# Shigangli/Ok-Topk

Measured on AMD Instinct MI355X. Metric: tokens/s (bert_base seq128 bs8/GPU, Ok-Topk density=0.001, step time & allreduce ms; speedup vs dense), higher is better.
Workload: dtype bf16; 1 GPU; model=bert_base, global_batch=8, seq_len=128, parallelism=dp1, compressor=oktopk, wire_dtype=bf16

## Files before the change

### oktopk_amd/allreducer.py

```python
from __future__ import annotations

import logging
import math
import time
from dataclasses import dataclass
from typing import Dict, List, Optional, Tuple

import torch

from . import ops
from .comm import Comm
from .config import EngineConfig

logger = logging.getLogger("oktopk_amd")

COMPRESSORS = [
    "none",
    "dense",
    "oktopk",
    "topkA",
    "topkA2",
    "topkAopt",
    "topkSA",
    "gtopk",
    "gaussiank",
    "gaussiankconcat",
    "gaussiankSA",
]


@dataclass
class TensorState:

    residual: torch.Tensor
    counter: int = 0
    tau_local: float = 0.0
    tau_global: float = 0.0
    boundaries: Optional[torch.Tensor] = None
    mask: Optional[torch.Tensor] = None
    grad_src: Optional[torch.Tensor] = None

    def state_dict(self) -> dict:
        return {
            "residual": self.residual,
            "counter": self.counter,
            "tau_local": self.tau_local,
            "tau_global": self.tau_global,
            "boundaries": self.boundaries,
        }

    def load_state_dict(self, d: dict) -> None:
        self.residual.copy_(d["residual"].to(self.residual.device))
        self.counter = int(d["counter"])
        self.tau_local = float(d["tau_local"])
        self.tau_global = float(d["tau_global"])
        self.boundaries = d["boundaries"]


class AllReducer:

    def __init__(self, comm: Comm, cfg: Optional[EngineConfig] = None):
        self.comm = comm
        self.cfg = cfg or EngineConfig()
        if self.cfg.compressor not in COMPRESSORS:
            raise ValueError(
                f"unknown compressor {self.cfg.compressor!r}; choose from {COMPRESSORS}"
            )
        self.states: Dict[str, TensorState] = {}
        self.timers: Dict[str, Dict[str, float]] = {}
        self.eps_log: List[Tuple[int, float]] = []
        self.randk_log: List[Tuple[int, float]] = []
        self.upbound_log: List[Tuple[int, float]] = []
        self.train_epoch = 0
        self.timing_sync = False

    def set_comm(self, comm: Comm) -> None:
        self.comm = comm
        for st in self.states.values():
            st.boundaries = None

    def state(self, name: str, t: torch.Tensor) -> TensorState:
        st = self.states.get(name)
        if st is None:
            st = TensorState(residual=torch.zeros_like(t))
            self.states[name] = st
        return st

    def _time(self, name: str, phase: str, dt: float) -> None:
        self.timers.setdefault(name, {}).setdefault(phase, 0.0)
        self.timers[name][phase] += dt

    def run(self, name: str, tensor: torch.Tensor,
            grad_src: Optional[torch.Tensor] = None) -> torch.Tensor:
        t = tensor.reshape(-1)
        if self.timing_sync and t.is_cuda:
            torch.cuda.synchronize()
        comp = self.cfg.compressor
        if comp == "oktopk" and self.cfg.oktopk.pipeline_chunks > 1:
            return self._oktopk_chunked(name, tensor, grad_src)
        st = self.state(name, t)
        ok = self.cfg.oktopk
        fused_ef = comp in ("oktopk", "topkAopt", "topkSA", "gaussiankSA") or (
            self.cfg.gaussian_device_select
            and comp in ("gaussiank", "gaussiankconcat"))
        if grad_src is not None and not (
            fused_ef and st.counter >= ok.dense_warmup_iters
        ):
            t.copy_(grad_src.reshape(-1).to(t.dtype))
            grad_src = None
        st.grad_src = grad_src

        eps_ref = None
        if self.cfg.profiling_norm and comp not in ("none", "dense"):
            if grad_src is not None:
                dense_in = grad_src.reshape(-1).to(t.dtype) + st.residual
            else:
                dense_in = t + st.residual
            eps_ref = self._dense_value(dense_in)
            k = self._k(t.numel())
            top = torch.topk(eps_ref.abs(), k)
            eps_topk = torch.zeros_like(eps_ref)
            eps_topk[top.indices] = eps_ref[top.indices]
            eps_den = max(ops.l2norm(eps_ref), 1e-30)
            eps_ref = (eps_topk, eps_den, eps_ref)

        if comp in ("none", "dense") or st.counter < ok.dense_warmup_iters:
            out = self._dense(name, t)
        elif comp == "oktopk":
            out = self._oktopk(name, t, st)
        elif comp in ("topkA", "topkA2"):
# ... 173 lines not shown
            recv = comm.alltoallv(
                comm.to_comm(send),
                [self._pack_ints(c) for c in elem_counts],
                [self._pack_ints(c) for c in recv_elems],
            )
            if not ok.device_wire:
                r_idx, r_val = self._unpack(recv, recv_elems)
        else:
            r_idx, r_val = idx, val
        self._time(name, "alltoall", time.perf_counter() - s1)

        s2 = time.perf_counter()
        exact = it % ok.global_threshold_recompute_interval == 0 or st.tau_global <= 0.0
        if P > 1:
            reduced = torch.zeros(hi - lo, dtype=t.dtype, device=t.device)
            if ok.device_wire:
                ops.unpack_scatter_add_(reduced, recv.to(t.device), recv_elems,
                                        lo, self._wire_bf16)
            elif r_idx.numel():
                ops.scatter_add_(reduced, r_idx.to(t.device) - lo, r_val.to(t.device))
            self._time(name, "reduce", time.perf_counter() - s2)

            s3 = time.perf_counter()
            if exact:
                gidx, gval = ops.compact_gt(reduced, 0.0)
            else:
                gidx, gval = ops.compact_gt(reduced, st.tau_global)
            gidx = gidx + lo
        else:
            self._time(name, "reduce", time.perf_counter() - s2)
            s3 = time.perf_counter()
            if not exact:
                result = t
                result.zero_()
                gsz = ops.scatter_gt_credit_(result, st.residual, idx, val,
                                             st.tau_global, 1.0)
                if gsz < ok.global_lo_num * k // ok.global_lo_den:
                    st.tau_global /= ok.scale_global_increase
                elif gsz > ok.global_hi_num * k // ok.global_hi_den:
                    st.tau_global *= ok.scale_global_decrease
                self._time(name, "allgather", time.perf_counter() - s3)
                return result
            gidx, gval = idx, val

        if P == 1:
            all_idx, all_val = gidx, gval
        elif ok.balanced_allgather:
            all_idx, all_val = self._balanced_round2(gidx, gval)
        elif ok.device_wire:
            pack = comm.to_comm(self._pack_one(gidx, gval, n))
            elem_counts = [int(x) for x in comm.allgather_sizes(gidx.numel(), comm.device)]
            buf, _ = comm.allgatherv(pack, sizes=[self._pack_ints(c) for c in elem_counts])
            all_idx, all_val = ops.unpack_segments(buf.to(t.device), elem_counts,
                                                   self._wire_bf16)
        else:
            pack = comm.to_comm(self._pack(gidx, gval))
            elem_counts = [int(x) for x in comm.allgather_sizes(gidx.numel(), comm.device)]
            buf, _ = comm.allgatherv(pack, sizes=[self._pack_ints(c) for c in elem_counts])
            all_idx, all_val = self._unpack(buf, elem_counts)
        all_idx = all_idx.to(t.device)
        all_val = all_val.to(t.device)
        self._time(name, "allgather", time.perf_counter() - s3)

        s4 = time.perf_counter()
        if exact:
            kk = min(k, all_val.numel())
            if kk > 0:
                top = torch.topk(all_val.abs(), kk, sorted=True)
                st.tau_global = float(top.values[-1].item())
                sel_pos = top.indices
                g_sel_idx = all_idx[sel_pos]
                g_sel_val = all_val[sel_pos]
            else:
                g_sel_idx = all_idx
                g_sel_val = all_val
        else:
            g_sel_idx = all_idx
            g_sel_val = all_val
            gsz = g_sel_idx.numel()
            if gsz < ok.global_lo_num * k // ok.global_lo_den:
                st.tau_global /= ok.scale_global_increase
            elif gsz > ok.global_hi_num * k // ok.global_hi_den:
                st.tau_global *= ok.scale_global_decrease

        result = t
        ops.fill_sparse_scaled_(result, g_sel_idx, g_sel_val, 1.0 / P)

        self._residual_credit(st, idx, g_sel_idx, n, t.device)
        self._time(name, "merge", time.perf_counter() - s4)
        return result

    def _residual_credit(self, st: TensorState, idx: torch.Tensor,
                         g_sel_idx: torch.Tensor, n: int, device) -> None:
        if idx.numel() and g_sel_idx.numel():
            if st.mask is None or st.mask.numel() != n:
                st.mask = torch.zeros(n, dtype=torch.bool, device=device)
            st.mask[g_sel_idx.long()] = True
            ops.zero_at_masked_(st.residual, idx, st.mask)
            st.mask[g_sel_idx.long()] = False

    def run_many(self, items: List[Tuple[str, torch.Tensor, Optional[torch.Tensor]]]) -> None:
        comp, ok = self.cfg.compressor, self.cfg.oktopk
        if (comp != "oktopk" or self.cfg.profiling_norm
                or ok.pipeline_chunks > 1 or ok.balanced_allgather
                or len(items) <= 1):
            for name, t, g in items:
                self.run(name, t, grad_src=g)
            return
        if self.timing_sync and items[0][1].is_cuda:
            torch.cuda.synchronize()
        parts, warm = [], []
        for name, tensor, g in items:
            t = tensor.reshape(-1)
            st = self.state(name, t)
            it = st.counter
            st.counter += 1
            if it < ok.dense_warmup_iters:
                if g is not None:
                    t.copy_(g.reshape(-1).to(t.dtype))
# ... 761 lines not shown
```

### oktopk_amd/ops/__init__.py

```python
from __future__ import annotations

import os
from typing import Tuple

import torch

from . import reference as _ref

_FORCE_TORCH = os.environ.get("OKTOPK_FORCE_TORCH_OPS", "0") == "1"
_hip = None
_hip_err: Exception | None = None


def _load_hip():
    global _hip, _hip_err
    if _hip is None and _hip_err is None:
        try:
            from oktopk_amd import _hip_ops

            _hip = _hip_ops
        except ImportError as e:
            _hip_err = e
    return _hip

# ... 94 lines not shown

def ef_restore_upcast_(t: torch.Tensor, residual: torch.Tensor, g: torch.Tensor) -> torch.Tensor:
    return _backend(t).ef_restore_upcast_(t, residual, g)


def fused_sgd_(param, grad, momentum_buf, lr, momentum, weight_decay, nesterov):
    return _backend(param).fused_sgd_(
        param, grad, momentum_buf, float(lr), float(momentum), float(weight_decay), bool(nesterov)
    )


def fused_adam_(param, grad, exp_avg, exp_avg_sq, lr, beta1, beta2, eps,
                weight_decay, gscale=None):
    return _backend(param).fused_adam_(
        param, grad, exp_avg, exp_avg_sq, float(lr), float(beta1), float(beta2),
        float(eps), float(weight_decay), gscale
    )


def fused_adam_mirror_(param, grad, exp_avg, exp_avg_sq, param_bf16, lr, beta1,
                       beta2, eps, weight_decay, gscale=None):
    b = _backend(param)
    if hasattr(b, "fused_adam_mirror_"):
        return b.fused_adam_mirror_(
            param, grad, exp_avg, exp_avg_sq, param_bf16, float(lr), float(beta1),
            float(beta2), float(eps), float(weight_decay), gscale
        )
    b.fused_adam_(param, grad, exp_avg, exp_avg_sq, float(lr), float(beta1),
                  float(beta2), float(eps), float(weight_decay), gscale)
    param_bf16.copy_(param)


def scatter_gt_credit_(result, residual, idx, val, tau, scale=1.0) -> int:
    return int(_backend(result).scatter_gt_credit_(
        result, residual, idx, val, float(tau), float(scale)))



def _wire_backend(t: torch.Tensor, nseg: int):
    b = _backend(t)
    if b is not _ref and nseg > b.wire_max_segments():
        return _ref
    return b


def pack_regions(idx: torch.Tensor, val: torch.Tensor, bounds: torch.Tensor,
                 wire_bf16: bool):
    buf, counts = _wire_backend(idx, bounds.numel() - 1).pack_regions(
        idx, val, bounds, bool(wire_bf16))
    return buf, [int(c) for c in counts]


def unpack_segments(buf: torch.Tensor, counts, wire_bf16: bool):
    counts = [int(c) for c in counts]
    idx, val = _wire_backend(buf, len(counts)).unpack_segments(
        buf, counts, bool(wire_bf16))
    return idx, val


def unpack_scatter_add_(dest: torch.Tensor, buf: torch.Tensor, counts,
                        base: int, wire_bf16: bool) -> torch.Tensor:
    counts = [int(c) for c in counts]
    return _wire_backend(dest, len(counts)).unpack_scatter_add_(
        dest, buf, counts, int(base), bool(wire_bf16))


def grad_clip_scale(t: torch.Tensor, max_norm: float) -> torch.Tensor:
    return _backend(t).grad_clip_scale(t, float(max_norm))
# ... 9 lines not shown
```

### oktopk_amd/ops/csrc/bindings.cpp

```cpp

#include <torch/extension.h>
#include <ATen/cuda/CUDAContext.h>
#include <ATen/cuda/CUDAGeneratorImpl.h>
#include <c10/cuda/CUDAGuard.h>

#include <cstdint>
#include <vector>

extern "C" {
void launch_count_gt(const float*, int64_t, float, unsigned long long*, hipStream_t);
void launch_count_multi_gt(const float*, int64_t, const float*, int, unsigned long long*,
                           hipStream_t);
void launch_compact_count_multi(const float*, int64_t, const float*, int, int64_t,
                                int, int*, hipStream_t);
void launch_compact_write(const float*, int64_t, float, int64_t, int, const int*,
                          int32_t*, float*, hipStream_t);
void launch_hist(const float*, int64_t, uint32_t, uint32_t, int, int, unsigned int*,
                 hipStream_t);
void launch_scatter_add(float*, const int32_t*, const float*, int64_t, hipStream_t);
void launch_scatter_set_scaled(float*, const int32_t*, const float*, float, int64_t,
                               hipStream_t);
void launch_scatter_gt_credit(const int32_t*, const float*, int64_t, float,
                              float, float*, float*, unsigned long long*,
                              hipStream_t);
void launch_zero_at(float*, const int32_t*, int64_t, hipStream_t);
void launch_zero_at_masked(float*, const int32_t*, const bool*, int64_t, hipStream_t);
void launch_isin_sorted(const int32_t*, int64_t, const int32_t*, int64_t, bool*,
                        hipStream_t);
void launch_ef_restore(float*, float*, int64_t, hipStream_t);
void launch_ef_upcast(float*, float*, const void*, int64_t, hipStream_t);
void launch_ef_count(float*, float*, const void*, int64_t, const float*, int,
                     int64_t, int, int*, hipStream_t);
void launch_count_totals(const int*, int, int, int64_t*, hipStream_t);
void launch_scan_offsets(const int*, int, int*, hipStream_t);
void launch_sgd(float*, const float*, float*, int64_t, float, float, float, int,
                hipStream_t);
void launch_clip_scale(const double*, float, float*, hipStream_t);
void launch_adam(float*, const float*, float*, float*, void*, const float*, int64_t, float, float,
                 float, float, float, hipStream_t);
void launch_sumsq(const float*, int64_t, double*, hipStream_t);
void launch_colsum_into_bf16(const void*, int64_t, int64_t, void*, int,
                             hipStream_t);
bool ln_bwd_supported(int64_t H);
int ln_bwd_blocks(int64_t rows);
void launch_ln_bwd_into(const void* gy, const void* x, const void* gamma,
                        const float* mean, const float* rstd, int64_t rows,
                        int64_t H, void* gx, float* ws, void* dgamma,
                        void* dbeta, int accumulate, hipStream_t);
void launch_attn_rowdot(const void*, const void*, int64_t, int64_t, int64_t,
                        float*, hipStream_t);
void launch_linear_gelu(const void*, const void*, const float*, void*, void*, int,
                        int, int, int, hipStream_t);
void launch_add_ln_fwd(const void*, const void*, const void*, const void*, void*,
                       void*, float*, float*, int64_t, int, float, hipStream_t);
void launch_add_ln_bwd(const void*, const void*, const float*, const float*,
                       const void*, void*, float*, float*, int64_t, int,
                       hipStream_t);
void launch_attn_fwd(const void*, const void*, void*, void*, void*, int, int,
                     float, float, unsigned long long, unsigned long long,
                     const void*, const void*, unsigned int, int, int,
                     hipStream_t);
void launch_attn_fwd_fa(const void*, const void*, void*, void*, int, int, int,
                        float, float, unsigned long long, unsigned long long,
                        const void*, const void*, unsigned int, int, int,
                        hipStream_t);
void launch_dropout_mask_mul(void*, int64_t, int64_t, unsigned long long,
                             unsigned long long, const void*, const void*,
                             unsigned int, int, float, hipStream_t);
void launch_attn_bwd_fa(const void*, const void*, const void*, const void*,
                        const void*, void*, int, int, int, float, float,
                        unsigned long long, unsigned long long, const void*,
                        const void*, unsigned int, int, int, hipStream_t);
void launch_gauss_moments(const float*, float*, const void*, int64_t, int64_t,
// ... 402 lines not shown
}

static int64_t scatter_gt_credit_(torch::Tensor result,
                                  torch::Tensor residual, torch::Tensor idx,
                                  torch::Tensor val, double tau,
                                  double scale) {
    check_f32_1d(result, "result");
    check_f32_1d(residual, "residual");
    check_f32_1d(val, "val");
    TORCH_CHECK(idx.scalar_type() == torch::kInt32 && idx.is_contiguous());
    const at::cuda::CUDAGuard guard(result.device());
    auto cnt = torch::zeros({1}, result.options().dtype(torch::kInt64));
    launch_scatter_gt_credit(idx.data_ptr<int32_t>(), val.data_ptr<float>(),
                             idx.numel(), (float)tau, (float)scale,
                             result.data_ptr<float>(),
                             residual.data_ptr<float>(),
                             (unsigned long long*)cnt.data_ptr<int64_t>(),
                             cur_stream());
    return cnt.cpu().item<int64_t>();
}

static torch::Tensor grad_clip_scale(torch::Tensor t, double max_norm) {
    check_f32_1d(t, "t");
    const at::cuda::CUDAGuard guard(t.device());
    auto ss = torch::zeros({1}, t.options().dtype(torch::kFloat64));
    launch_sumsq(t.data_ptr<float>(), t.numel(), ss.data_ptr<double>(),
                 cur_stream());
    auto out = torch::empty({1}, t.options());
    launch_clip_scale(ss.data_ptr<double>(), (float)max_norm,
                      out.data_ptr<float>(), cur_stream());
    return out;
}

static void colsum_bf16_into(torch::Tensor gy, torch::Tensor dst,
                             bool accumulate) {
    TORCH_CHECK(gy.is_cuda() && gy.scalar_type() == torch::kBFloat16 &&
                gy.is_contiguous() && gy.dim() >= 1, "gy: contiguous cuda bf16");
    TORCH_CHECK(dst.is_cuda() && dst.scalar_type() == torch::kBFloat16 &&
                dst.is_contiguous() && dst.device() == gy.device(),
                "dst: contiguous cuda bf16 on gy's device");
    int64_t C = gy.size(-1);
    TORCH_CHECK(dst.numel() == C, "dst must hold gy.size(-1) elements");
    if (C == 0) return;
    int64_t R = gy.numel() / C;
    const at::cuda::CUDAGuard guard(gy.device());
    launch_colsum_into_bf16(gy.data_ptr(), R, C, dst.data_ptr(),
                            accumulate ? 1 : 0, cur_stream());
}

static torch::Tensor linear_bwd_into(torch::Tensor gy, torch::Tensor x,
                                     torch::Tensor w,
                                     c10::optional<torch::Tensor> gw_dst,
                                     c10::optional<torch::Tensor> gb_dst,
                                     bool accumulate, bool bias_kernel) {
    TORCH_CHECK(gy.is_cuda() && gy.scalar_type() == torch::kBFloat16 &&
                x.scalar_type() == torch::kBFloat16 &&
                w.scalar_type() == torch::kBFloat16 && w.dim() == 2,
                "linear_bwd_into: cuda bf16 operands");
    const int64_t N = w.size(0), K = w.size(1);
    TORCH_CHECK(gy.size(-1) == N && x.size(-1) == K &&
                gy.numel() / std::max<int64_t>(N, 1) ==
                    x.numel() / std::max<int64_t>(K, 1),
                "linear_bwd_into: shape mismatch");
    const at::cuda::CUDAGuard guard(gy.device());
    at::NoGradGuard no_grad;
    auto gy2 = gy.contiguous().view({-1, N});
// ... 469 lines not shown
          "fused EF restore(+bf16 upcast) + adaptive-threshold compaction",
          py::arg("t"), py::arg("residual"), py::arg("grad"), py::arg("taus"),
          py::arg("hi_limit"));
    m.def("gaussian_select_ef", &gaussian_select_ef,
          "device-resident Gaussian-k selection: EF restore + fp64 moments, "
          "on-device ppf + refine tree, compact write; returns (idx, val, "
          "chosen, count, tau, tau0, mean, std)",
          py::arg("t"), py::arg("residual"), py::arg("grad"),
          py::arg("density"), py::arg("k"));
    m.def("kth_abs_value", &kth_abs_value, "exact k-th largest |t| via radix select");
    m.def("scatter_add_", &scatter_add_, "dest[idx] += val");
    m.def("zero_at_", &zero_at_, "t[idx] = 0");
    m.def("zero_at_masked_", &zero_at_masked_, "t[idx[i]] = 0 where mask[idx[i]]");
    m.def("fill_sparse_scaled_", &fill_sparse_scaled_, "out=0; out[idx]=val*scale");
    m.def("isin_sorted", &isin_sorted, "membership of a in sorted b");
    m.def("ef_restore_snapshot_", &ef_restore_snapshot_, "t+=r; r=t (fused)");
    m.def("ef_restore_upcast_", &ef_restore_upcast_,
          "t = float(g_bf16) + r; r = t (fused upcast + EF restore)");
    m.def("fused_sgd_", &fused_sgd_, "fused SGD step");
    m.def("fused_adam_", &fused_adam_, "fused (Bert)Adam step",
          py::arg("p"), py::arg("g"), py::arg("m"), py::arg("v"),
          py::arg("lr"), py::arg("b1"), py::arg("b2"), py::arg("eps"),
          py::arg("wd"), py::arg("gscale") = py::none());
    m.def("fused_adam_mirror_", &fused_adam_mirror_,
          "fused Adam step + bf16 weight-mirror write",
          py::arg("p"), py::arg("g"), py::arg("m"), py::arg("v"),
          py::arg("p_bf16"), py::arg("lr"), py::arg("b1"), py::arg("b2"),
          py::arg("eps"), py::arg("wd"), py::arg("gscale") = py::none());
    m.def("scatter_gt_credit_", &scatter_gt_credit_,
          "fused world-1 round-2 tail: result[idx]=val*scale and "
          "residual[idx]=0 where |val|>tau; returns the count");
    m.def("grad_clip_scale", &grad_clip_scale,
          "device-resident clip factor min(1, max/||t||) (no host sync)");
    m.def("l2norm", &l2norm, "L2 norm (fp64 accumulate)");
    m.def("colsum_bf16_into", &colsum_bf16_into,
          "bias grad: dst (=|+=) column sum of bf16 [R, C], one launch",
          py::arg("gy"), py::arg("dst"), py::arg("accumulate") = false);
    m.def("ln_bwd_supported", &ln_bwd_into_supported,
          "hidden sizes ln_bwd_into handles");
    m.def("ln_bwd_into", &ln_bwd_into,
          "LayerNorm backward; dgamma/dbeta written into their gradient slots, returns gx",
          py::arg("gy"), py::arg("x"), py::arg("gamma"), py::arg("mean"),
          py::arg("rstd"), py::arg("dgamma_dst"), py::arg("dbeta_dst"),
          py::arg("accumulate") = false);
    m.def("linear_bwd_into", &linear_bwd_into,
          "Linear backward; gW/gb written into their gradient slots, returns gx",
          py::arg("gy"), py::arg("x"), py::arg("w"), py::arg("gw_dst"),
          py::arg("gb_dst"), py::arg("accumulate") = false,
          py::arg("bias_kernel") = false);
    m.def("attn_rowdot", &attn_rowdot,
          "flash-bwd D: per-(head,row) dot of gO and O (head_dim 64)");
    m.def("sumsq_into_", &sumsq_into_,
          "accumulate sum(t^2) into a device fp64[1] (no host sync)");
    m.def("attn_fwd", &attn_fwd,
          "fused self-attention forward: softmax(QK^T*scale+mask) dropout @ V "
          "(bf16 MFMA, seq=128/hd=64; returns ctx [+P, A for backward])");
    m.def("attn_fwd_fa", &attn_fwd_fa,
          "flash (online-softmax) attention forward: any seq % 128 == 0, "
          "hd=64 bf16; returns (ctx, lse, philox_state) — O(S) memory");
    m.def("attn_bwd_fa", &attn_bwd_fa,
          "flash attention backward: dQ/dK/dV from (qkv, gO, lse, D) with "
          "philox dropout-mask regeneration — nothing O(S^2) materialised");
    m.def("dropout_mask_mul_", &dropout_mask_mul_,
          "regenerate the forward's philox dropout mask in-place: "
          "a[i] = keep ? a[i]/keep_prob : 0");
    m.def("wire_max_segments", []() { return (int64_t)wire_max_segments(); },
// ... 18 lines not shown
```

### oktopk_amd/ops/csrc/kernels.hip

```cpp

#include <hip/hip_runtime.h>
#include <cstdint>

#define BLOCK 256
#define WAVES_PER_BLOCK (BLOCK / 64)
#define MAX_BLOCKS 2048

static inline uint32_t tau_to_bits(float tau) {
    if (tau < 0.f) return 0xFFFFFFFFu;
    union { float f; uint32_t u; } c;
    c.f = tau;
    return c.u & 0x7fffffffu;
}

__device__ __forceinline__ bool sel_gt(uint32_t abits, uint32_t tau_bits) {
    return (tau_bits == 0xFFFFFFFFu) | (abits > tau_bits);
}

static inline int n_blocks(int64_t work, int per_thread = 1) {
    int64_t b = (work + (int64_t)BLOCK * per_thread - 1) / ((int64_t)BLOCK * per_thread);
    if (b < 1) b = 1;
    if (b > MAX_BLOCKS) b = MAX_BLOCKS;
    return (int)b;
}
// ... 305 lines not shown
                                      const bool* mask, int64_t m,
                                      hipStream_t stream) {
    hipLaunchKernelGGL(zero_at_masked_kernel, dim3(n_blocks(m, 4)), dim3(BLOCK), 0,
                       stream, dest, idx, mask, m);
}

__global__ void zero_at_kernel(float* __restrict__ dest,
                               const int32_t* __restrict__ idx, int64_t m) {
    int64_t i = (int64_t)blockIdx.x * BLOCK + threadIdx.x;
    int64_t stride = (int64_t)gridDim.x * BLOCK;
    for (; i < m; i += stride) dest[idx[i]] = 0.f;
}

extern "C" void launch_zero_at(float* dest, const int32_t* idx, int64_t m,
                               hipStream_t stream) {
    hipLaunchKernelGGL(zero_at_kernel, dim3(n_blocks(m, 4)), dim3(BLOCK), 0, stream,
                       dest, idx, m);
}

__global__ void scatter_gt_credit_kernel(const int32_t* __restrict__ idx,
                                         const float* __restrict__ val,
                                         int64_t m, uint32_t tau_bits,
                                         float scale,
                                         float* __restrict__ result,
                                         float* __restrict__ residual,
                                         unsigned long long* __restrict__ cnt) {
    int64_t i = (int64_t)blockIdx.x * BLOCK + threadIdx.x;
    int64_t stride = (int64_t)gridDim.x * BLOCK;
    unsigned long long c = 0;
    for (; i < m; i += stride) {
        float v = val[i];
        if (sel_gt(abs_bits(v), tau_bits)) {
            int32_t j = idx[i];
            result[j] = v * scale;
            residual[j] = 0.f;
            ++c;
        }
    }
    for (int off = 32; off > 0; off >>= 1) c += __shfl_down(c, off, 64);
    __shared__ unsigned long long ws[WAVES_PER_BLOCK];
    int lane = threadIdx.x & 63, wave = threadIdx.x >> 6;
    if (lane == 0) ws[wave] = c;
    __syncthreads();
    if (threadIdx.x == 0) {
        unsigned long long s = 0;
        for (int w = 0; w < WAVES_PER_BLOCK; ++w) s += ws[w];
        atomicAdd(cnt, s);
    }
}

extern "C" void launch_scatter_gt_credit(const int32_t* idx, const float* val,
                                         int64_t m, float tau, float scale,
                                         float* result, float* residual,
                                         unsigned long long* cnt,
                                         hipStream_t stream) {
    hipLaunchKernelGGL(scatter_gt_credit_kernel, dim3(n_blocks(m, 4)),
                       dim3(BLOCK), 0, stream, idx, val, m, tau_to_bits(tau),
                       scale, result, residual, cnt);
}

__global__ void isin_sorted_kernel(const int32_t* __restrict__ a, int64_t m,
                                   const int32_t* __restrict__ b, int64_t nb,
                                   bool* __restrict__ out) {
    int64_t i = (int64_t)blockIdx.x * BLOCK + threadIdx.x;
    int64_t stride = (int64_t)gridDim.x * BLOCK;
    for (; i < m; i += stride) {
        int32_t x = a[i];
// ... 350 lines not shown
                             double* __restrict__ out) {
    const float4* t4 = reinterpret_cast<const float4*>(t);
    int64_t i = (int64_t)blockIdx.x * BLOCK + threadIdx.x;
    int64_t stride = (int64_t)gridDim.x * BLOCK;
    double acc = 0.0;
    for (; i < n4; i += stride) {
        float4 v = t4[i];
        acc += (double)v.x * v.x + (double)v.y * v.y
             + (double)v.z * v.z + (double)v.w * v.w;
    }
    for (i = n4 * 4 + (int64_t)blockIdx.x * BLOCK + threadIdx.x; i < n; i += stride) {
        double x = t[i];
        acc += x * x;
    }
    for (int off = 32; off > 0; off >>= 1)
        acc += __shfl_down(acc, off, 64);
    __shared__ double ws[WAVES_PER_BLOCK];
    int lane = threadIdx.x & 63, wave = threadIdx.x >> 6;
    if (lane == 0) ws[wave] = acc;
    __syncthreads();
    if (threadIdx.x == 0) {
        double s = 0;
        for (int w = 0; w < WAVES_PER_BLOCK; ++w) s += ws[w];
        atomicAdd(out, s);
    }
}

extern "C" void launch_sumsq(const float* t, int64_t n, double* out, hipStream_t stream) {
    int64_t n4 = ((uintptr_t)t & 15) == 0 ? n >> 2 : 0;
    hipLaunchKernelGGL(sumsq_kernel, dim3(n_blocks(n, 8)), dim3(BLOCK), 0, stream,
                       t, n, n4, out);
}

__device__ __forceinline__ float ks_b2f(short u) {
    union { float f; uint32_t i; } c;
    c.i = ((uint32_t)(uint16_t)u) << 16;
    return c.f;
}

__global__ void attn_rowdot_kernel(const short* __restrict__ go,
                                   const short* __restrict__ out,
                                   int64_t B, int64_t S, int64_t NH,
                                   float* __restrict__ d) {
    int64_t row = ((int64_t)blockIdx.x * (BLOCK / 64)) + (threadIdx.x >> 6);
    int lane = threadIdx.x & 63;
    int64_t nrows = B * NH * S;
    if (row >= nrows) return;
    int64_t s = row % S;
    int64_t bh = row / S;
    int64_t b = bh / NH, h = bh % NH;
    int64_t off = ((b * S + s) * NH + h) * 64 + lane;
    float v = ks_b2f(go[off]) * ks_b2f(out[off]);
    for (int o = 32; o > 0; o >>= 1) v += __shfl_down(v, o, 64);
    if (lane == 0) d[row] = v;
}

extern "C" void launch_attn_rowdot(const void* go, const void* out, int64_t B,
                                   int64_t S, int64_t NH, float* d,
                                   hipStream_t stream) {
    int64_t nrows = B * NH * S;
    int64_t blocks = (nrows + (BLOCK / 64) - 1) / (BLOCK / 64);
    hipLaunchKernelGGL(attn_rowdot_kernel, dim3((unsigned)blocks), dim3(BLOCK),
                       0, stream, (const short*)go, (const short*)out, B, S,
                       NH, d);
}
```

### oktopk_amd/ops/reference.py

```python
from __future__ import annotations

from typing import Tuple

import torch

__all__ = [
    "kth_abs_value",
    "compact_gt",
    "count_gt",
    "count_multi_gt",
    "compact_adaptive",
    "gaussian_select_ef",
    "scatter_add_",
    "zero_at_",
    "zero_at_masked_",
    "fill_sparse_scaled_",
    "isin_sorted",
    "ef_restore_snapshot_",
    "ef_restore_upcast_",
    "fused_sgd_",
    "fused_adam_",
    "l2norm",
    "pack_regions",
    "unpack_segments",
# ... 165 lines not shown
    param.add_(d_p, alpha=-lr)


def fused_adam_(
    param: torch.Tensor,
    grad: torch.Tensor,
    exp_avg: torch.Tensor,
    exp_avg_sq: torch.Tensor,
    lr: float,
    beta1: float,
    beta2: float,
    eps: float,
    weight_decay: float,
    gscale=None,
) -> None:
    if gscale is not None:
        grad = grad * gscale.to(grad.device, grad.dtype)
    exp_avg.mul_(beta1).add_(grad, alpha=1 - beta1)
    exp_avg_sq.mul_(beta2).addcmul_(grad, grad, value=1 - beta2)
    update = exp_avg / (exp_avg_sq.sqrt() + eps)
    if weight_decay != 0:
        update = update + weight_decay * param
    param.add_(update, alpha=-lr)


def scatter_gt_credit_(result, residual, idx, val, tau, scale=1.0) -> int:
    sel = val.abs() > tau
    j = idx.long()[sel]
    result[j] = val[sel] * scale
    residual[j] = 0.0
    return int(sel.sum())



def _wire_words(c: int, wire_bf16: bool) -> int:
    return c + (c + 1) // 2 if wire_bf16 else 2 * c


def pack_regions(idx: torch.Tensor, val: torch.Tensor, bounds: torch.Tensor,
                 wire_bf16: bool):
    P = bounds.numel() - 1
    m = idx.numel()
    cuts = [0, m]
    if P > 1:
        split = torch.searchsorted(idx.long(), bounds[1:P].to(idx.device)).cpu()
        cuts = [0] + [int(x) for x in split] + [m]
    counts = [cuts[j + 1] - cuts[j] for j in range(P)]
    segs = []
    for j in range(P):
        i, v = idx[cuts[j]:cuts[j + 1]], val[cuts[j]:cuts[j + 1]]
        if wire_bf16:
            v = v.to(torch.bfloat16)
            if v.numel() % 2:
                v = torch.cat([v, v.new_zeros(1)])
        segs += [i.view(torch.int32), v.view(torch.int32)]
    return torch.cat(segs), counts


def unpack_segments(buf: torch.Tensor, counts, wire_bf16: bool):
    idxs, vals = [], []
    off = 0
    for n in counts:
        ints = _wire_words(n, wire_bf16)
        idxs.append(buf[off:off + n])
        if wire_bf16:
            vals.append(buf[off + n:off + ints].view(torch.bfloat16)[:n].float())
# ... 30 lines not shown
```

### oktopk_amd/optimizer.py

```python
from __future__ import annotations

import math
import queue
import threading
from typing import Dict, Iterable, List, Optional, Tuple

import torch

from . import ops
from .allreducer import AllReducer
from .comm import Comm
from .config import EngineConfig

__all__ = ["DistributedOptimizer", "FlatBertAdam", "SCHEDULES"]



def warmup_cosine(x: float, warmup: float = 0.002) -> float:
    if x < warmup:
        return x / warmup
    return 0.5 * (1.0 + math.cos(math.pi * x))


def warmup_constant(x: float, warmup: float = 0.002) -> float:
    if x < warmup:
        return x / warmup
    return 1.0


def warmup_linear(x: float, warmup: float = 0.002) -> float:
    if x < warmup:
        return x / warmup
    return max((x - 1.0) / (warmup - 1.0), 0.0)


# ... 422 lines not shown
            self._plan_zero_ranges()

    def set_substep(self, sub: int) -> None:
        if sub == 0 and self._dg_owner is not None:
            self._settle_direct_grad()
            self._dg_owner.written.clear()

    def zero_grad(self, set_to_none: bool = False):
        self._settle_direct_grad()
        if self._zero_ranges is None:
            self.flat_grad_model.zero_()
        else:
            for a, b in self._zero_ranges:
                self.flat_grad_model[a:b].zero_()
        for p, (o, n_) in zip(self.params, self.slots):
            p.grad = self.flat_grad_model[o : o + n_].view_as(p)

    @property
    def param_groups(self):
        return [{"lr": self.lr, "params": self.params}]

    def current_lr(self) -> float:
        if self.t_total > 0:
            return self.lr * self.schedule(self.step_count / self.t_total, self.warmup)
        return self.lr

    def get_lr(self) -> list:
        if self.step_count == 0:
            return [0]
        return [self.current_lr()]

    def step(self):
        self._settle_direct_grad()
        if self.cfg.compressor in ("dense", "none") and self.model_dtype != torch.float32:
            self.reducer.run("flat", self.flat_grad_model)
            self.flat_grad.copy_(self.flat_grad_model)
        elif self.flat_grad_model is not self.flat_grad:
            self.reducer.run("flat", self.flat_grad, grad_src=self.flat_grad_model)
        else:
            self.reducer.run("flat", self.flat_grad)
        gscale = None
        if self.max_grad_norm and self.max_grad_norm > 0:
            gscale = ops.grad_clip_scale(self.flat_grad, self.max_grad_norm)
        lr = self.current_lr()
        b1, b2 = self.betas
        d = self.decay_numel
        mirrored = self.flat_param_model is not self.flat_param
        def _adam(sl, wd):
            if mirrored:
                ops.fused_adam_mirror_(
                    self.flat_param[sl], self.flat_grad[sl], self.exp_avg[sl],
                    self.exp_avg_sq[sl], self.flat_param_model[sl], lr, b1, b2,
                    self.eps, wd, gscale=gscale,
                )
            else:
                ops.fused_adam_(
                    self.flat_param[sl], self.flat_grad[sl], self.exp_avg[sl],
                    self.exp_avg_sq[sl], lr, b1, b2, self.eps, wd,
                    gscale=gscale,
                )
        if d > 0:
            _adam(slice(None, d), self.weight_decay)
        if d < self.numel:
            _adam(slice(d, None), 0.0)
        self.step_count += 1

    def sync_master_from_model(self) -> None:
        if self.flat_param_model is not self.flat_param:
            self.flat_param.copy_(self.flat_param_model)

    def state_dict(self):
        return {
            "step_count": self.step_count,
            "flat_param": self.flat_param,
            "exp_avg": self.exp_avg,
            "exp_avg_sq": self.exp_avg_sq,
            "reducer": {n: s.state_dict() for n, s in self.reducer.states.items()},
        }

    def load_state_dict(self, d):
        self.step_count = int(d["step_count"])
        if "flat_param" in d:
# ... 17 lines not shown
```

Before: 134,700 tokens/s.

## Feed sparse gradient directly into fused Adam, skipping dense gradient materialization

When Ok-Topk produces a thresholded sparse result, the reducer now hands (idx, val, scale, tau) to the optimizer instead of zeroing and scattering into the dense flat gradient. New kernels compute the grad-clip norm from the sparse values and run a fused Adam that looks up per-tile sparse entries via a binary-searched tile_start table. This removes a full-length zero fill, the scatter, and the dense norm read. In exchange it adds a tile-start search kernel and per-element scans over the sparse entries in each tile, and flat_grad no longer holds the reduced gradient.

```diff
diff --git a/oktopk_amd/allreducer.py b/oktopk_amd/allreducer.py
--- a/oktopk_amd/allreducer.py
+++ b/oktopk_amd/allreducer.py
@@ -55,6 +55,15 @@
         self.tau_local = float(d["tau_local"])
         self.tau_global = float(d["tau_global"])
         self.boundaries = d["boundaries"]
+
+
+@dataclass
+class SparseGrad:
+
+    idx: torch.Tensor
+    val: torch.Tensor
+    scale: float
+    tau: float
 
 
 class AllReducer:
@@ -73,6 +82,8 @@
         self.upbound_log: List[Tuple[int, float]] = []
         self.train_epoch = 0
         self.timing_sync = False
+        self.sparse_result: Optional[SparseGrad] = None
+        self._sparse_ok = False
 
     def set_comm(self, comm: Comm) -> None:
         self.comm = comm
@@ -91,11 +102,14 @@
         self.timers[name][phase] += dt
 
     def run(self, name: str, tensor: torch.Tensor,
-            grad_src: Optional[torch.Tensor] = None) -> torch.Tensor:
+            grad_src: Optional[torch.Tensor] = None,
+            sparse_ok: bool = False) -> torch.Tensor:
         t = tensor.reshape(-1)
         if self.timing_sync and t.is_cuda:
             torch.cuda.synchronize()
         comp = self.cfg.compressor
+        self.sparse_result = None
+        self._sparse_ok = bool(sparse_ok) and not self.cfg.profiling_norm
         if comp == "oktopk" and self.cfg.oktopk.pipeline_chunks > 1:
             return self._oktopk_chunked(name, tensor, grad_src)
         st = self.state(name, t)
@@ -335,9 +349,15 @@
             s3 = time.perf_counter()
             if not exact:
                 result = t
-                result.zero_()
-                gsz = ops.scatter_gt_credit_(result, st.residual, idx, val,
-                                             st.tau_global, 1.0)
+                if self._sparse_ok:
+                    self.sparse_result = SparseGrad(idx, val, 1.0,
+                                                    st.tau_global)
+                    gsz = ops.scatter_gt_credit_(None, st.residual, idx, val,
+                                                 st.tau_global)
+                else:
+                    result.zero_()
+                    gsz = ops.scatter_gt_credit_(result, st.residual, idx,
+                                                 val, st.tau_global, 1.0)
                 if gsz < ok.global_lo_num * k // ok.global_lo_den:
                     st.tau_global /= ok.scale_global_increase
                 elif gsz > ok.global_hi_num * k // ok.global_hi_den:
@@ -387,7 +407,12 @@
                 st.tau_global *= ok.scale_global_decrease
 
         result = t
-        ops.fill_sparse_scaled_(result, g_sel_idx, g_sel_val, 1.0 / P)
+        if (self._sparse_ok and not exact and P > 1
+                and not ok.balanced_allgather):
+            self.sparse_result = SparseGrad(
+                g_sel_idx.to(torch.int32), g_sel_val, 1.0 / P, -1.0)
+        else:
+            ops.fill_sparse_scaled_(result, g_sel_idx, g_sel_val, 1.0 / P)
 
         self._residual_credit(st, idx, g_sel_idx, n, t.device)
         self._time(name, "merge", time.perf_counter() - s4)
diff --git a/oktopk_amd/ops/__init__.py b/oktopk_amd/ops/__init__.py
--- a/oktopk_amd/ops/__init__.py
+++ b/oktopk_amd/ops/__init__.py
@@ -150,8 +150,50 @@
 
 
 def scatter_gt_credit_(result, residual, idx, val, tau, scale=1.0) -> int:
+    if result is None:
+        return int(_backend(residual).credit_gt_(residual, idx, val, float(tau)))
     return int(_backend(result).scatter_gt_credit_(
         result, residual, idx, val, float(tau), float(scale)))
+
+
+
+def sparse_sumsq_into_(acc: torch.Tensor, idx, val, scale: float,
+                       tau: float) -> None:
+    return _backend(val).sparse_sumsq_into_(acc, idx, val, float(scale),
+                                            float(tau))
+
+
+def grad_clip_scale_sparse(idx, val, scale: float, tau: float,
+                           max_norm: float, n: int) -> torch.Tensor:
+    b = _backend(val)
+    if b is _ref:
+        return b.grad_clip_scale_sparse(idx, val, float(scale), float(tau),
+                                        float(max_norm), int(n))
+    return b.grad_clip_scale_sparse(idx, val, float(scale), float(tau),
+                                    float(max_norm))
+
+
+def fused_adam_sparse_(param, idx, val, base, scale, tau, exp_avg, exp_avg_sq,
+                       lr, beta1, beta2, eps, weight_decay, gscale=None):
+    return _backend(param).fused_adam_sparse_(
+        param, idx, val, int(base), float(scale), float(tau), exp_avg,
+        exp_avg_sq, float(lr), float(beta1), float(beta2), float(eps),
+        float(weight_decay), gscale)
+
+
+def fused_adam_sparse_mirror_(param, idx, val, base, scale, tau, exp_avg,
+                              exp_avg_sq, param_bf16, lr, beta1, beta2, eps,
+                              weight_decay, gscale=None):
+    b = _backend(param)
+    if hasattr(b, "fused_adam_sparse_mirror_"):
+        return b.fused_adam_sparse_mirror_(
+            param, idx, val, int(base), float(scale), float(tau), exp_avg,
+            exp_avg_sq, param_bf16, float(lr), float(beta1), float(beta2),
+            float(eps), float(weight_decay), gscale)
+    b.fused_adam_sparse_(param, idx, val, int(base), float(scale), float(tau),
+                         exp_avg, exp_avg_sq, float(lr), float(beta1),
+                         float(beta2), float(eps), float(weight_decay), gscale)
+    param_bf16.copy_(param)
 
 
 
diff --git a/oktopk_amd/ops/csrc/bindings.cpp b/oktopk_amd/ops/csrc/bindings.cpp
--- a/oktopk_amd/ops/csrc/bindings.cpp
+++ b/oktopk_amd/ops/csrc/bindings.cpp
@@ -39,6 +39,12 @@
 void launch_adam(float*, const float*, float*, float*, void*, const float*, int64_t, float, float,
                  float, float, float, hipStream_t);
 void launch_sumsq(const float*, int64_t, double*, hipStream_t);
+void launch_sparse_sumsq(const float*, int64_t, float, float, double*, hipStream_t);
+int64_t adam_sparse_ntiles(int64_t);
+void launch_adam_sparse(float*, float*, float*, void*, const float*, int64_t,
+                        const int32_t*, const float*, int64_t, int32_t*, int64_t,
+                        float, float, float, float, float, float, float,
+                        hipStream_t);
 void launch_colsum_into_bf16(const void*, int64_t, int64_t, void*, int,
                              hipStream_t);
 bool ln_bwd_supported(int64_t H);
@@ -507,6 +513,100 @@
     return out;
 }
 
+
+static void check_sparse_grad(const torch::Tensor& idx, const torch::Tensor& val) {
+    check_i32_1d(idx, "idx");
+    check_f32_1d(val, "val");
+    TORCH_CHECK(idx.numel() == val.numel(), "idx / val length mismatch");
+    TORCH_CHECK(idx.numel() < (int64_t)INT32_MAX, "selection too large");
+}
+
+static int64_t credit_gt_(torch::Tensor residual, torch::Tensor idx,
+                          torch::Tensor val, double tau) {
+    check_f32_1d(residual, "residual");
+    check_sparse_grad(idx, val);
+    const at::cuda::CUDAGuard guard(residual.device());
+    auto cnt = torch::zeros({1}, residual.options().dtype(torch::kInt64));
+    launch_scatter_gt_credit(idx.data_ptr<int32_t>(), val.data_ptr<float>(),
+                             idx.numel(), (float)tau, 1.f, nullptr,
+                             residual.data_ptr<float>(),
+                             (unsigned long long*)cnt.data_ptr<int64_t>(),
+                             cur_stream());
+    return cnt.cpu().item<int64_t>();
+}
+
+static void sparse_sumsq_into_(torch::Tensor acc, torch::Tensor idx,
+                               torch::Tensor val, double scale, double tau) {
+    check_sparse_grad(idx, val);
+    TORCH_CHECK(acc.is_cuda() && acc.scalar_type() == torch::kFloat64 &&
+                acc.numel() == 1 && acc.device() == val.device(),
+                "acc must be a 1-elem fp64 tensor on val's device");
+    const at::cuda::CUDAGuard guard(val.device());
+    launch_sparse_sumsq(val.data_ptr<float>(), val.numel(), (float)scale,
+                        (float)tau, acc.data_ptr<double>(), cur_stream());
+}
+
+static torch::Tensor grad_clip_scale_sparse(torch::Tensor idx, torch::Tensor val,
+                                            double scale, double tau,
+                                            double max_norm) {
+    check_sparse_grad(idx, val);
+    const at::cuda::CUDAGuard guard(val.device());
+    auto ss = torch::zeros({1}, val.options().dtype(torch::kFloat64));
+    launch_sparse_sumsq(val.data_ptr<float>(), val.numel(), (float)scale,
+                        (float)tau, ss.data_ptr<double>(), cur_stream());
+    auto out = torch::empty({1}, val.options());
+    launch_clip_scale(ss.data_ptr<double>(), (float)max_norm,
+                      out.data_ptr<float>(), cur_stream());
+    return out;
+}
+
+static void adam_sparse_impl(torch::Tensor& p, torch::Tensor& idx,
+                             torch::Tensor& val, int64_t base, double scale,
+                             double tau, torch::Tensor& m, torch::Tensor& v,
+                             void* p_bf16, double lr, double b1, double b2,
+                             double eps, double wd,
+                             const c10::optional<torch::Tensor>& gscale) {
+    check_f32_1d(p, "p");
+    check_f32_1d(m, "m");
+    check_f32_1d(v, "v");
+    check_sparse_grad(idx, val);
+    TORCH_CHECK(m.numel() == p.numel() && v.numel() == p.numel(),
+                "p / m / v length mismatch");
+    TORCH_CHECK(base >= 0, "base must be >= 0");
+    const at::cuda::CUDAGuard guard(p.device());
+    auto tile_start = torch::empty({adam_sparse_ntiles(p.numel()) + 1},
+                                   idx.options());
+    launch_adam_sparse(p.data_ptr<float>(), m.data_ptr<float>(),
+                       v.data_ptr<float>(), p_bf16, gscale_ptr(gscale),
+                       p.numel(), idx.data_ptr<int32_t>(), val.data_ptr<float>(),
+                       idx.numel(), tile_start.data_ptr<int32_t>(), base,
+                       (float)scale, (float)tau, (float)lr, (float)b1,
+                       (float)b2, (float)eps, (float)wd, cur_stream());
+}
+
+static void fused_adam_sparse_(torch::Tensor p, torch::Tensor idx,
+                               torch::Tensor val, int64_t base, double scale,
+                               double tau, torch::Tensor m, torch::Tensor v,
+                               double lr, double b1, double b2, double eps,
+                               double wd, c10::optional<torch::Tensor> gscale) {
+    adam_sparse_impl(p, idx, val, base, scale, tau, m, v, nullptr, lr, b1, b2,
+                     eps, wd, gscale);
+}
+
+static void fused_adam_sparse_mirror_(torch::Tensor p, torch::Tensor idx,
+                                      torch::Tensor val, int64_t base,
+                                      double scale, double tau, torch::Tensor m,
+                                      torch::Tensor v, torch::Tensor p_bf16,
+                                      double lr, double b1, double b2,
+                                      double eps, double wd,
+                                      c10::optional<torch::Tensor> gscale) {
+    TORCH_CHECK(p_bf16.is_cuda() && p_bf16.scalar_type() == torch::kBFloat16 &&
+                p_bf16.is_contiguous() && p_bf16.numel() == p.numel(),
+                "p_bf16: contiguous cuda bf16 of p's length");
+    adam_sparse_impl(p, idx, val, base, scale, tau, m, v, p_bf16.data_ptr(), lr,
+                     b1, b2, eps, wd, gscale);
+}
+
 static void colsum_bf16_into(torch::Tensor gy, torch::Tensor dst,
                              bool accumulate) {
     TORCH_CHECK(gy.is_cuda() && gy.scalar_type() == torch::kBFloat16 &&
@@ -1042,6 +1142,24 @@
           "residual[idx]=0 where |val|>tau; returns the count");
     m.def("grad_clip_scale", &grad_clip_scale,
           "device-resident clip factor min(1, max/||t||) (no host sync)");
+    m.def("credit_gt_", &credit_gt_,
+          "residual[idx]=0 where |val|>tau; returns the count (no dense result)");
+    m.def("sparse_sumsq_into_", &sparse_sumsq_into_,
+          "acc (fp64[1]) += sum((val*scale)^2) over entries with |val|>tau");
+    m.def("grad_clip_scale_sparse", &grad_clip_scale_sparse,
+          "grad_clip_scale of a sparse gradient (idx, val, scale, tau)");
+    m.def("fused_adam_sparse_", &fused_adam_sparse_,
+          "fused Adam step, gradient given as (idx, val, base, scale, tau)",
+          py::arg("p"), py::arg("idx"), py::arg("val"), py::arg("base"),
+          py::arg("scale"), py::arg("tau"), py::arg("m"), py::arg("v"),
+          py::arg("lr"), py::arg("b1"), py::arg("b2"), py::arg("eps"),
+          py::arg("wd"), py::arg("gscale") = py::none());
+    m.def("fused_adam_sparse_mirror_", &fused_adam_sparse_mirror_,
+          "fused_adam_sparse_ + bf16 weight-mirror write",
+          py::arg("p"), py::arg("idx"), py::arg("val"), py::arg("base"),
+          py::arg("scale"), py::arg("tau"), py::arg("m"), py::arg("v"),
+          py::arg("p_bf16"), py::arg("lr"), py::arg("b1"), py::arg("b2"),
+          py::arg("eps"), py::arg("wd"), py::arg("gscale") = py::none());
     m.def("l2norm", &l2norm, "L2 norm (fp64 accumulate)");
     m.def("colsum_bf16_into", &colsum_bf16_into,
           "bias grad: dst (=|+=) column sum of bf16 [R, C], one launch",
diff --git a/oktopk_amd/ops/csrc/kernels.hip b/oktopk_amd/ops/csrc/kernels.hip
--- a/oktopk_amd/ops/csrc/kernels.hip
+++ b/oktopk_amd/ops/csrc/kernels.hip
@@ -361,7 +361,7 @@
         float v = val[i];
         if (sel_gt(abs_bits(v), tau_bits)) {
             int32_t j = idx[i];
-            result[j] = v * scale;
+            if (result) result[j] = v * scale;
             residual[j] = 0.f;
             ++c;
         }
@@ -778,6 +778,178 @@
                        t, n, n4, out);
 }
 
+#define ADAM_TILE (BLOCK * 4)
+
+__global__ void sparse_sumsq_kernel(const float* __restrict__ val, int64_t m,
+                                    float scale, uint32_t tau_bits,
+                                    double* __restrict__ out) {
+    int64_t i = (int64_t)blockIdx.x * BLOCK + threadIdx.x;
+    int64_t stride = (int64_t)gridDim.x * BLOCK;
+    double acc = 0.0;
+    for (; i < m; i += stride) {
+        float x = val[i];
+        if (sel_gt(abs_bits(x), tau_bits)) {
+            float g = x * scale;
+            acc += (double)g * g;
+        }
+    }
+    for (int off = 32; off > 0; off >>= 1)
+        acc += __shfl_down(acc, off, 64);
+    __shared__ double ws[WAVES_PER_BLOCK];
+    int lane = threadIdx.x & 63, wave = threadIdx.x >> 6;
+    if (lane == 0) ws[wave] = acc;
+    __syncthreads();
+    if (threadIdx.x == 0) {
+        double s = 0;
+        for (int w = 0; w < WAVES_PER_BLOCK; ++w) s += ws[w];
+        atomicAdd(out, s);
+    }
+}
+
+extern "C" void launch_sparse_sumsq(const float* val, int64_t m, float scale,
+                                    float tau, double* out, hipStream_t stream) {
+    if (m <= 0) return;
+    hipLaunchKernelGGL(sparse_sumsq_kernel, dim3(n_blocks(m, 4)), dim3(BLOCK), 0,
+                       stream, val, m, scale, tau_to_bits(tau), out);
+}
+
+__global__ void sparse_tile_start_kernel(const int32_t* __restrict__ idx,
+                                         int64_t m, int64_t base, int64_t n,
+                                         int64_t ntiles,
+                                         int32_t* __restrict__ tile_start) {
+    int64_t t = (int64_t)blockIdx.x * BLOCK + threadIdx.x;
+    int64_t stride = (int64_t)gridDim.x * BLOCK;
+    for (; t <= ntiles; t += stride) {
+        int64_t off = t * ADAM_TILE;
+        if (off > n) off = n;
+        int64_t target = base + off;
+        int64_t lo = 0, hi = m;
+        while (lo < hi) {
+            int64_t mid = (lo + hi) >> 1;
+            if ((int64_t)idx[mid] < target) lo = mid + 1; else hi = mid;
+        }
+        tile_start[t] = (int32_t)lo;
+    }
+}
+
+template <bool VEC>
+__device__ __forceinline__ float adam_one_as_compiled(float pi, float gi,
+                                                      float& mi, float& vi,
+                                                      float lr, float b1,
+                                                      float b2, float eps,
+                                                      float wd) {
+#pragma clang fp contract(off)
+    const float c1 = 1.f - b1, c2 = 1.f - b2;
+    if (VEC) {
+        mi = __builtin_fmaf(c1, gi, mi * b1);
+        vi = __builtin_fmaf(c2 * gi, gi, vi * b2);
+    } else {
+        mi = __builtin_fmaf(mi, b1, c1 * gi);
+        vi = __builtin_fmaf(vi, b2, (c2 * gi) * gi);
+    }
+    const float up = __builtin_fmaf(wd, pi, mi / (sqrtf(vi) + eps));
+    return __builtin_fmaf(-lr, up, pi);
+}
+
+__global__ void adam_sparse_kernel(float* __restrict__ p, float* __restrict__ m,
+                                   float* __restrict__ v,
+                                   short* __restrict__ p_bf16,
+                                   const float* __restrict__ gscale_ptr,
+                                   int64_t n, int64_t n4,
+                                   const int32_t* __restrict__ idx,
+                                   const float* __restrict__ val,
+                                   const int32_t* __restrict__ tile_start,
+                                   int64_t base, float scale, uint32_t tau_bits,
+                                   float lr, float b1, float b2, float eps,
+                                   float wd) {
+    const float gs = gscale_ptr ? *gscale_ptr : 1.f;
+    float4* p4 = reinterpret_cast<float4*>(p);
+    float4* m4 = reinterpret_cast<float4*>(m);
+    float4* v4 = reinterpret_cast<float4*>(v);
+    short4* b4 = reinterpret_cast<short4*>(p_bf16);
+    const int64_t nt4 = (n4 + BLOCK - 1) / BLOCK;
+    int64_t T = blockIdx.x;
+    int hs = 0, he = 0;
+    if (T < nt4) { hs = tile_start[T]; he = tile_start[T + 1]; }
+    for (; T < nt4; T += gridDim.x) {
+        const int64_t Tn = T + gridDim.x;
+        int hs_n = 0, he_n = 0;
+        if (Tn < nt4) { hs_n = tile_start[Tn]; he_n = tile_start[Tn + 1]; }
+        const int64_t i = T * BLOCK + threadIdx.x;
+        if (i < n4) {
+            float4 pi = p4[i], mi = m4[i], vi = v4[i];
+            float4 gi = make_float4(0.f, 0.f, 0.f, 0.f);
+            const int64_t e0 = base + 4 * i;
+            for (int h = hs; h < he; ++h) {
+                const float x = val[h];
+                const int64_t j = (int64_t)idx[h] - e0;
+                const bool keep = sel_gt(abs_bits(x), tau_bits);
+                const float g = x * scale;
+                gi.x = (keep & (j == 0)) ? g : gi.x;
+                gi.y = (keep & (j == 1)) ? g : gi.y;
+                gi.z = (keep & (j == 2)) ? g : gi.z;
+                gi.w = (keep & (j == 3)) ? g : gi.w;
+            }
+            pi.x = adam_one_as_compiled<true>(pi.x, gi.x * gs, mi.x, vi.x,
+                                             lr, b1, b2, eps, wd);
+            pi.y = adam_one_as_compiled<true>(pi.y, gi.y * gs, mi.y, vi.y,
+                                             lr, b1, b2, eps, wd);
+            pi.z = adam_one_as_compiled<true>(pi.z, gi.z * gs, mi.z, vi.z,
+                                             lr, b1, b2, eps, wd);
+            pi.w = adam_one_as_compiled<true>(pi.w, gi.w * gs, mi.w, vi.w,
+                                             lr, b1, b2, eps, wd);
+            m4[i] = mi; v4[i] = vi; p4[i] = pi;
+            if (p_bf16)
+                b4[i] = make_short4(adam_f2b(pi.x), adam_f2b(pi.y),
+                                    adam_f2b(pi.z), adam_f2b(pi.w));
+        }
+        hs = hs_n; he = he_n;
+    }
+    const int64_t stride = (int64_t)gridDim.x * BLOCK;
+    for (int64_t i = n4 * 4 + (int64_t)blockIdx.x * BLOCK + threadIdx.x; i < n;
+         i += stride) {
+        const int64_t T = i / ADAM_TILE;
+        const int hs = tile_start[T], he = tile_start[T + 1];
+        const int64_t e0 = base + i;
+        float gi = 0.f;
+        for (int h = hs; h < he; ++h) {
+            const float x = val[h];
+            if ((int64_t)idx[h] == e0 && sel_gt(abs_bits(x), tau_bits))
+                gi = x * scale;
+        }
+        float mi = m[i], vi = v[i];
+        float pn = adam_one_as_compiled<false>(p[i], gi * gs, mi, vi, lr, b1, b2,
+                                                eps, wd);
+        m[i] = mi; v[i] = vi; p[i] = pn;
+        if (p_bf16) p_bf16[i] = adam_f2b(pn);
+    }
+}
+
+extern "C" int64_t adam_sparse_ntiles(int64_t n) {
+    return (n + ADAM_TILE - 1) / ADAM_TILE;
+}
+
+extern "C" void launch_adam_sparse(float* p, float* m, float* v, void* p_bf16,
+                                   const float* gscale, int64_t n,
+                                   const int32_t* idx, const float* val,
+                                   int64_t m_entries, int32_t* tile_start,
+                                   int64_t base, float scale, float tau,
+                                   float lr, float b1, float b2, float eps,
+                                   float wd, hipStream_t stream) {
+    if (n <= 0) return;
+    int64_t ntiles = adam_sparse_ntiles(n);
+    hipLaunchKernelGGL(sparse_tile_start_kernel, dim3(n_blocks(ntiles + 1)),
+                       dim3(BLOCK), 0, stream, idx, m_entries, base, n, ntiles,
+                       tile_start);
+    bool aligned = (((uintptr_t)p | (uintptr_t)m | (uintptr_t)v) & 15) == 0 &&
+                   (((uintptr_t)p_bf16) & 7) == 0;
+    int64_t n4 = aligned ? n >> 2 : 0;
+    hipLaunchKernelGGL(adam_sparse_kernel, dim3(n_blocks(n, 8)), dim3(BLOCK), 0,
+                       stream, p, m, v, (short*)p_bf16, gscale, n, n4, idx, val,
+                       tile_start, base, scale, tau_to_bits(tau), lr, b1, b2,
+                       eps, wd);
+}
+
 __device__ __forceinline__ float ks_b2f(short u) {
     union { float f; uint32_t i; } c;
     c.i = ((uint32_t)(uint16_t)u) << 16;
diff --git a/oktopk_amd/ops/reference.py b/oktopk_amd/ops/reference.py
--- a/oktopk_amd/ops/reference.py
+++ b/oktopk_amd/ops/reference.py
@@ -221,6 +221,46 @@
     return int(sel.sum())
 
 
+def credit_gt_(residual, idx, val, tau) -> int:
+    sel = val.abs() > tau
+    residual[idx.long()[sel]] = 0.0
+    return int(sel.sum())
+
+
+
+def _sparse_kept(val: torch.Tensor, tau: float) -> torch.Tensor:
+    if tau < 0:
+        return torch.ones_like(val, dtype=torch.bool)
+    return val.abs() > tau
+
+
+def densify_sparse_grad(idx, val, base: int, n: int, scale: float, tau: float):
+    g = torch.zeros(n, dtype=torch.float32, device=val.device)
+    j = idx.long() - int(base)
+    keep = _sparse_kept(val, tau) & (j >= 0) & (j < n)
+    g[j[keep]] = val[keep] * scale
+    return g
+
+
+def sparse_sumsq_into_(acc: torch.Tensor, idx, val, scale: float,
+                       tau: float) -> None:
+    g = val[_sparse_kept(val, tau)] * scale
+    acc += (g.double() ** 2).sum()
+
+
+def grad_clip_scale_sparse(idx, val, scale: float, tau: float,
+                           max_norm: float, n: int) -> torch.Tensor:
+    return grad_clip_scale(densify_sparse_grad(idx, val, 0, n, scale, tau),
+                           max_norm)
+
+
+def fused_adam_sparse_(param, idx, val, base, scale, tau, exp_avg, exp_avg_sq,
+                       lr, beta1, beta2, eps, weight_decay, gscale=None) -> None:
+    g = densify_sparse_grad(idx, val, base, param.numel(), scale, tau)
+    fused_adam_(param, g, exp_avg, exp_avg_sq, lr, beta1, beta2, eps,
+                weight_decay, gscale)
+
+
 
 def _wire_words(c: int, wire_bf16: bool) -> int:
     return c + (c + 1) // 2 if wire_bf16 else 2 * c
diff --git a/oktopk_amd/optimizer.py b/oktopk_amd/optimizer.py
--- a/oktopk_amd/optimizer.py
+++ b/oktopk_amd/optimizer.py
@@ -1,6 +1,7 @@
 from __future__ import annotations
 
 import math
+import os
 import queue
 import threading
 from typing import Dict, Iterable, List, Optional, Tuple
@@ -489,22 +490,46 @@
 
     def step(self):
         self._settle_direct_grad()
+        sparse_ok = os.environ.get("OKTOPK_SPARSE_STEP", "1") != "0"
+        self.reducer.sparse_result = None
         if self.cfg.compressor in ("dense", "none") and self.model_dtype != torch.float32:
             self.reducer.run("flat", self.flat_grad_model)
             self.flat_grad.copy_(self.flat_grad_model)
         elif self.flat_grad_model is not self.flat_grad:
-            self.reducer.run("flat", self.flat_grad, grad_src=self.flat_grad_model)
+            self.reducer.run("flat", self.flat_grad, grad_src=self.flat_grad_model,
+                             sparse_ok=sparse_ok)
         else:
-            self.reducer.run("flat", self.flat_grad)
+            self.reducer.run("flat", self.flat_grad, sparse_ok=sparse_ok)
+        sg = self.reducer.sparse_result
         gscale = None
         if self.max_grad_norm and self.max_grad_norm > 0:
-            gscale = ops.grad_clip_scale(self.flat_grad, self.max_grad_norm)
+            if sg is not None:
+                gscale = ops.grad_clip_scale_sparse(
+                    sg.idx, sg.val, sg.scale, sg.tau, self.max_grad_norm,
+                    self.numel)
+            else:
+                gscale = ops.grad_clip_scale(self.flat_grad, self.max_grad_norm)
         lr = self.current_lr()
         b1, b2 = self.betas
         d = self.decay_numel
         mirrored = self.flat_param_model is not self.flat_param
         def _adam(sl, wd):
-            if mirrored:
+            if sg is not None:
+                base = sl.start or 0
+                if mirrored:
+                    ops.fused_adam_sparse_mirror_(
+                        self.flat_param[sl], sg.idx, sg.val, base, sg.scale,
+                        sg.tau, self.exp_avg[sl], self.exp_avg_sq[sl],
+                        self.flat_param_model[sl], lr, b1, b2, self.eps, wd,
+                        gscale=gscale,
+                    )
+                else:
+                    ops.fused_adam_sparse_(
+                        self.flat_param[sl], sg.idx, sg.val, base, sg.scale,
+                        sg.tau, self.exp_avg[sl], self.exp_avg_sq[sl], lr, b1,
+                        b2, self.eps, wd, gscale=gscale,
+                    )
+            elif mirrored:
                 ops.fused_adam_mirror_(
                     self.flat_param[sl], self.flat_grad[sl], self.exp_avg[sl],
                     self.exp_avg_sq[sl], self.flat_param_model[sl], lr, b1, b2,
```

Measured after the change: 139,600 tokens/s, median of 6. 3.6% higher.
